# argmaxinc/DiffusionKit

Hardware: NVIDIA H100
Metric: images/sec at 1024x1024 (FLUX.1-schnell 4-step) (higher is better)
Workload: dtype bf16

## Files before the change

### diffusionkit_b200/csrc/common.cuh

```cuda
#pragma once

#include <cuda.h>
#include <cuda_bf16.h>
#include <cuda_fp16.h>
#include <cuda_runtime.h>
#include <stdint.h>
#include <stdio.h>

#include "wgmma.cuh"

namespace dk {

__device__ __forceinline__ uint32_t smem_u32(const void* p) {
  return static_cast<uint32_t>(__cvta_generic_to_shared(p));
}


#ifndef DK_WATCHDOG_CYCLES
#define DK_WATCHDOG_CYCLES (8000000000LL)
#endif

__device__ __forceinline__ void mbar_init(uint64_t* bar, uint32_t count) {
  asm volatile("mbarrier.init.shared::cta.b64 [%0], %1;" ::"r"(smem_u32(bar)), "r"(count) : "memory");
}
// ... 14 lines not shown
      "mbarrier.try_wait.parity.shared::cta.b64 p, [%1], %2;\n\t"
      "selp.u32 %0, 1, 0, p;\n\t}"
      : "=r"(ok)
      : "r"(smem_u32(bar)), "r"(parity)
      : "memory");
  return ok;
}
#ifndef DK_WATCHDOG_SPINS
#define DK_WATCHDOG_SPINS (1u << 26)
#endif
static __device__ __noinline__ void mbar_watchdog_trap(uint64_t* bar, uint32_t parity) {
  printf("[dkb200] mbarrier watchdog: block (%d,%d,%d) thread %d bar@%u parity %u\n", blockIdx.x, blockIdx.y, blockIdx.z,
         threadIdx.x, smem_u32(bar), parity);
  __trap();
}
__device__ __forceinline__ void mbar_wait(uint64_t* bar, uint32_t parity) {
  if (mbar_try_wait(bar, parity)) return;
  uint32_t spins = 0;
  while (!mbar_try_wait(bar, parity)) {
    if (++spins == DK_WATCHDOG_SPINS) mbar_watchdog_trap(bar, parity);
  }
}


__device__ __forceinline__ void mbar_wait_warp(uint64_t* bar, uint32_t parity) {
  if ((threadIdx.x & 31) == 0) mbar_wait(bar, parity);
  __syncwarp();
}

__device__ __forceinline__ void fence_proxy_async_smem() {
  asm volatile("fence.proxy.async.shared::cta;" ::: "memory");
}

__device__ __forceinline__ void named_bar_sync(uint32_t id, uint32_t nthreads) {
  asm volatile("bar.sync %0, %1;" ::"r"(id), "r"(nthreads) : "memory");
}

__device__ __forceinline__ void tma_prefetch_desc(const CUtensorMap* m) {
  asm volatile("prefetch.tensormap [%0];" ::"l"(reinterpret_cast<uint64_t>(m)) : "memory");
}
__device__ __forceinline__ void tma_load_2d(void* dst, const CUtensorMap* map, uint64_t* bar, int c0, int c1) {
  asm volatile(
      "cp.async.bulk.tensor.2d.shared::cluster.global.tile.mbarrier::complete_tx::bytes [%0], [%1, {%3, %4}], [%2];" ::
          "r"(smem_u32(dst)),
      "l"(reinterpret_cast<uint64_t>(map)), "r"(smem_u32(bar)), "r"(c0), "r"(c1)
      : "memory");
}
__device__ __forceinline__ void tma_load_4d(void* dst, const CUtensorMap* map, uint64_t* bar, int c0, int c1, int c2,
                                            int c3) {
  asm volatile(
      "cp.async.bulk.tensor.4d.shared::cluster.global.tile.mbarrier::complete_tx::bytes [%0], [%1, {%3, %4, %5, %6}], "
      "[%2];" ::"r"(smem_u32(dst)),
      "l"(reinterpret_cast<uint64_t>(map)), "r"(smem_u32(bar)), "r"(c0), "r"(c1), "r"(c2), "r"(c3)
      : "memory");
}

__device__ __forceinline__ void wgmma_fence() { asm volatile("wgmma.fence.sync.aligned;" ::: "memory"); }
__device__ __forceinline__ void wgmma_commit() { asm volatile("wgmma.commit_group.sync.aligned;" ::: "memory"); }
template <int N>
__device__ __forceinline__ void wgmma_wait() {
  asm volatile("wgmma.wait_group.sync.aligned %0;" ::"n"(N) : "memory");
}
template <int N>
__device__ __forceinline__ void reg_fence(float (&d)[N]) {
#pragma unroll
  for (int i = 0; i < N; ++i) asm volatile("" : "+f"(d[i])::"memory");
}

// ... 104 lines not shown
```

### diffusionkit_b200/csrc/gemm.cu

```cuda
#include <stdlib.h>

#include "common.cuh"
#include "gemm_epilogue.cuh"
#include "host.h"

namespace dk {

constexpr int BM = 128;
constexpr int BK = 64;
constexpr int GEMM_THREADS = 384;

template <int BN>
struct GemmCfg {
  static constexpr int STAGES = (BN == 256) ? 4 : (BN == 128 ? 6 : 8);
  static constexpr int A_BYTES = BM * BK * 2;
  static constexpr int B_BYTES = BN * BK * 2;
  static constexpr int PIPE_BYTES = STAGES * (A_BYTES + B_BYTES);
  static constexpr int STAGE_LD = BN + 4;
  static_assert(PIPE_BYTES >= BM * STAGE_LD * 4, "the epilogue staging tile reuses the pipeline buffers");
  static constexpr int BAR_BYTES = 256;
  static constexpr int SMEM_BYTES = PIPE_BYTES + BAR_BYTES + 1024;
};

template <typename T, int BN, bool B_MN, int MODE>
__global__ void __launch_bounds__(GEMM_THREADS, 1)
gemm_wgmma_kernel(const __grid_constant__ CUtensorMap tmA, const __grid_constant__ CUtensorMap tmB, const GemmShape s,
                  const GemmEpi e, const ConvGeom g) {
  using Cfg = GemmCfg<BN>;
  constexpr int STAGES = Cfg::STAGES;
  constexpr int A_BYTES = Cfg::A_BYTES;
  constexpr int B_BYTES = Cfg::B_BYTES;

  extern __shared__ uint8_t smem_raw[];
  uint8_t* smem = smem_raw + ((1024u - (smem_u32(smem_raw) & 1023u)) & 1023u);
  uint8_t* sA = smem;
  uint8_t* sB = smem + STAGES * A_BYTES;
  uint64_t* full_bar = reinterpret_cast<uint64_t*>(smem + Cfg::PIPE_BYTES);
  uint64_t* empty_bar = full_bar + STAGES;

  const int warp = threadIdx.x >> 5;
  const int lane = threadIdx.x & 31;
  const int wg = threadIdx.x >> 7;

  if (threadIdx.x == 0) {
    tma_prefetch_desc(&tmA);
    tma_prefetch_desc(&tmB);
    for (int i = 0; i < STAGES; ++i) {
      mbar_init(&full_bar[i], 1);
      mbar_init(&empty_bar[i], 8);
    }
    fence_barrier_init();
  }
  __syncthreads();

  constexpr int GM = 16;
  int m_blk, n_blk;
  {
    const int tile = blockIdx.x;
    const int group_size = GM * s.num_n;
    const int group = tile / group_size;
    const int first_m = group * GM;
    const int gsz = min(s.num_m - first_m, GM);
    const int in_group = tile - group * group_size;
    m_blk = first_m + in_group % gsz;
    n_blk = in_group / gsz;
  }

  if (wg == 0) {
    if (warp != 0) return;
    int img = 0, y0 = 0, x0 = 0;
    if (MODE == 1) {
      const int per_img = g.tiles_x * g.tiles_y;
      img = m_blk / per_img;
      const int t = m_blk - img * per_img;
      y0 = (t / g.tiles_x) * g.TH;
      x0 = (t % g.tiles_x) * g.TW;
    }
    uint32_t stage = 0, phase = 0;
    for (int kb = 0; kb < s.num_k; ++kb) {
      mbar_wait_warp(&empty_bar[stage], phase ^ 1);
      if (elect_one_sync()) {
        mbar_arrive_expect_tx(&full_bar[stage], A_BYTES + B_BYTES);
        uint8_t* a_dst = sA + stage * A_BYTES;
        uint8_t* b_dst = sB + stage * B_BYTES;
        if (MODE == 0) {
          tma_load_2d(a_dst, &tmA, &full_bar[stage], kb * BK, m_blk * BM);
        } else {
          const int tap = kb / g.cblocks;
          const int c0 = (kb - tap * g.cblocks) * BK;
          const int dy = tap / 3, dx = tap - dy * 3;
          tma_load_4d(a_dst, &tmA, &full_bar[stage], c0, x0 * g.stride + dx - g.pad, y0 * g.stride + dy - g.pad, img);
        }
        if (!B_MN) {
          tma_load_2d(b_dst, &tmB, &full_bar[stage], kb * BK, n_blk * BN);
        } else {
#pragma unroll
          for (int j = 0; j < BN / 64; ++j)
            tma_load_2d(b_dst + j * (BK * 128), &tmB, &full_bar[stage], n_blk * BN + j * 64, kb * BK);
        }
      }
      __syncwarp();
      if (++stage == STAGES) {
        stage = 0;
        phase ^= 1;
      }
    }
    return;
  }

  const int cw = wg - 1;
  float acc[BN / 2];
#pragma unroll
  for (int i = 0; i < BN / 2; ++i) acc[i] = 0.f;
  {
    uint32_t stage = 0, phase = 0, prev = 0;
    for (int kb = 0; kb < s.num_k; ++kb) {
      mbar_wait(&full_bar[stage], phase);
      const uint32_t a_base = smem_u32(sA + stage * A_BYTES) + cw * 64 * 128;
      const uint32_t b_base = smem_u32(sB + stage * B_BYTES);
      wgmma_fence();
#pragma unroll
      for (int k = 0; k < BK / 16; ++k) {
        const uint64_t da = make_smem_desc_sw128(a_base + k * 32, 16, 1024);
        const uint64_t db = B_MN ? make_smem_desc_sw128(b_base + k * 16 * 128, BK * 128, 1024)
                                 : make_smem_desc_sw128(b_base + k * 32, 16, 1024);
        Wgmma<BN, Half16<T>::is_bf16, B_MN ? 1 : 0>::ss(acc, da, db, (kb | k) != 0 ? 1u : 0u);
      }
      wgmma_commit();
      wgmma_wait<1>();
      if (kb > 0 && lane == 0) mbar_arrive(&empty_bar[prev]);
      prev = stage;
      if (++stage == STAGES) {
        stage = 0;
        phase ^= 1;
      }
    }
    wgmma_wait<0>();
    reg_fence(acc);
  }

  float* stg = reinterpret_cast<float*>(smem);
  named_bar_sync(1, 256);
  stage_acc_rows<BN>(stg, Cfg::STAGE_LD, cw * 64, acc);
  named_bar_sync(1, 256);

  const int ew = warp - 4;
  const int quarter = ew & 3;
  const int half = ew >> 2;
  constexpr int NCH = BN / 64;
  const int r_in_tile = quarter * 32 + lane;

  bool row_ok;
  long long orow, rrow;
  int batch, pos = 0;
  if (MODE == 0) {
    const int m = m_blk * BM + r_in_tile;
    row_ok = m < s.M;
    batch = m / e.rpb;
    const int in_b = m - batch * e.rpb;
    pos = e.out_row_off + in_b;
    orow = static_cast<long long>(batch) * e.out_batch_rows + e.out_row_off + in_b;
    rrow = static_cast<long long>(batch) * e.res_batch_rows + e.res_row_off + in_b;
  } else {
    const int per_img = g.tiles_x * g.tiles_y;
    const int img = m_blk / per_img;
    const int t = m_blk - img * per_img;
    const int y = (t / g.tiles_x) * g.TH + r_in_tile / g.TW;
    const int x = (t % g.tiles_x) * g.TW + r_in_tile % g.TW;
    row_ok = (y < g.H) && (x < g.W);
    batch = img;
    orow = (static_cast<long long>(img) * g.H + y) * g.W + x;
    rrow = orow;
  }
  const float* srow = stg + r_in_tile * Cfg::STAGE_LD + half * (BN / 2);
  auto load32 = [&](int c, uint32_t (&r)[32]) {
#pragma unroll
    for (int q = 0; q < 8; ++q) {
      const float4 v = *reinterpret_cast<const float4*>(srow + c + 4 * q);
      r[4 * q] = __float_as_uint(v.x);
      r[4 * q + 1] = __float_as_uint(v.y);
      r[4 * q + 2] = __float_as_uint(v.z);
      r[4 * q + 3] = __float_as_uint(v.w);
    }
  };
  gemm_epilogue_drain<T, NCH, MODE>(s, e, load32, n_blk * BN + half * (BN / 2), row_ok, orow, rrow, batch, pos);
}

template <typename T, int BN, bool B_MN, int MODE>
static int launch_gemm_inst(dk_ctx* ctx, const CUtensorMap& tmA, const CUtensorMap& tmB, const GemmShape& s,
                            const GemmEpi& e, const ConvGeom& g, cudaStream_t stream) {
  using Cfg = GemmCfg<BN>;
  auto kern = gemm_wgmma_kernel<T, BN, B_MN, MODE>;
  static bool configured = false;
  if (!configured) {
    DK_CHECK_CUDA(cudaFuncSetAttribute(kern, cudaFuncAttributeMaxDynamicSharedMemorySize, Cfg::SMEM_BYTES));
    configured = true;
  }
  kern<<<s.num_m * s.num_n, GEMM_THREADS, Cfg::SMEM_BYTES, stream>>>(tmA, tmB, s, e, g);
  DK_LAUNCH_CHECK(ctx);
  return 0;
}

template <typename T, bool B_MN, int MODE>
static int launch_gemm_bn(dk_ctx* ctx, int bn, const CUtensorMap& tmA, const CUtensorMap& tmB, const GemmShape& s,
                          const GemmEpi& e, const ConvGeom& g, cudaStream_t stream) {
  if (bn == 256) return launch_gemm_inst<T, 256, B_MN, MODE>(ctx, tmA, tmB, s, e, g, stream);
  if (bn == 128) return launch_gemm_inst<T, 128, B_MN, MODE>(ctx, tmA, tmB, s, e, g, stream);
  return launch_gemm_inst<T, 64, B_MN, MODE>(ctx, tmA, tmB, s, e, g, stream);
}

static int pick_bn(const dk_ctx* ctx, int num_m, int N) {
  if (N <= 64) return 64;
  if (N <= 128) return 128;
  const int tiles256 = num_m * dk_ceil_div(N, 256);
  if (tiles256 >= ctx->sm_count) return 256;
  const int tiles128 = num_m * dk_ceil_div(N, 128);
  if (tiles128 >= ctx->sm_count || N % 256 != 0) return 128;
  return (tiles256 * 2 > ctx->sm_count) ? 256 : 128;
}

static bool aligned16(const void* p) { return (reinterpret_cast<uintptr_t>(p) & 15u) == 0; }
// ... 18 lines not shown
  GemmShape s = {};
  s.M = a->M;
  s.N = a->N;
  s.K = a->K;
  s.num_m = dk_ceil_div(a->M, BM);
  s.num_k = dk_ceil_div(a->K, BK);
  const int bn = a->w_n_major ? 128 : (a->qk_head_dim != 0 ? 256 : pick_bn(ctx, s.num_m, a->N));
  s.num_n = dk_ceil_div(a->N, bn);

  GemmEpi e;
  e.out = a->out;
  e.ldc = a->ldc;
  e.bias = a->bias;
  e.gate = a->gate;
  e.gate_ld = a->gate_ld;
  e.res = a->res;
  e.ldres = a->ldres;
  e.rpb = a->rows_per_batch > 0 ? a->rows_per_batch : a->M;
  e.out_batch_rows = a->rows_per_batch > 0 ? a->out_batch_rows : a->M;
  e.out_row_off = a->out_row_off;
  e.res_batch_rows = a->rows_per_batch > 0 ? a->res_batch_rows : a->M;
  e.res_row_off = a->res_row_off;
  e.act = a->act;
  {
    static const int dbg = [] { const char* v = getenv("DK_GEMM_EPI_DEBUG"); return v ? atoi(v) : 0; }();
    e.debug = dbg;
  }
  e.qk_qw = a->qk_q_weight;
  e.qk_kw = a->qk_k_weight;
  e.qk_rope = a->qk_rope;
  e.qk_d = a->qk_head_dim;
  e.qk_h = a->qk_heads * a->qk_head_dim;
  e.qk_eps = a->qk_eps;
  if (e.qk_d != 0) {
    DK_REQUIRE(e.qk_d == 64 || e.qk_d == 128, "dk_gemm: fused QK norm/RoPE supports head dims 64 and 128 (got %d)", e.qk_d);
    DK_REQUIRE(a->N == 3 * e.qk_h && e.qk_h % 128 == 0, "dk_gemm: fused QK epilogue needs N == 3*heads*d, heads*d %% 128 == 0");
    DK_REQUIRE(!a->w_n_major && a->act == DK_ACT_NONE && a->gate == nullptr && a->res == nullptr,
               "dk_gemm: fused QK epilogue excludes act/gate/residual");
    DK_REQUIRE(a->qk_rope == nullptr || (reinterpret_cast<uintptr_t>(a->qk_rope) & 15u) == 0, "dk_gemm: rope table alignment");
  }
  ConvGeom g = {};

  CUtensorMap tmA, tmB;
  {
    const uint64_t dims[2] = {static_cast<uint64_t>(a->K), static_cast<uint64_t>(a->M)};
    const uint64_t strides[1] = {static_cast<uint64_t>(a->lda) * 2};
    const uint32_t box[2] = {BK, BM};
    if (int rc = dk_make_tmap_16b(ctx, &tmA, a->A, 2, dims, strides, box)) return rc;
  }
  if (!a->w_n_major) {
    const uint64_t dims[2] = {static_cast<uint64_t>(a->K), static_cast<uint64_t>(a->N)};
    const uint64_t strides[1] = {static_cast<uint64_t>(a->ldw) * 2};
    const uint32_t box[2] = {BK, static_cast<uint32_t>(bn)};
    if (int rc = dk_make_tmap_16b(ctx, &tmB, a->W, 2, dims, strides, box)) return rc;
  } else {
    const uint64_t dims[2] = {static_cast<uint64_t>(a->N), static_cast<uint64_t>(a->K)};
    const uint64_t strides[1] = {static_cast<uint64_t>(a->ldw) * 2};
    const uint32_t box[2] = {64, BK};
    if (int rc = dk_make_tmap_16b(ctx, &tmB, a->W, 2, dims, strides, box)) return rc;
  }

  if (a->dtype == DK_BF16) {
    if (a->w_n_major) return launch_gemm_inst<__nv_bfloat16, 128, true, 0>(ctx, tmA, tmB, s, e, g, stream);
    return launch_gemm_bn<__nv_bfloat16, false, 0>(ctx, bn, tmA, tmB, s, e, g, stream);
  } else {
    if (a->w_n_major) return launch_gemm_inst<__half, 128, true, 0>(ctx, tmA, tmB, s, e, g, stream);
    return launch_gemm_bn<__half, false, 0>(ctx, bn, tmA, tmB, s, e, g, stream);
  }
}

static int conv3x3_impl(dk_ctx* ctx, int dtype, const void* x, const void* w, const void* bias, const void* res,
                        void* out, int B, int Hin, int Win, int Cin, int Cout, int stride, cudaStream_t stream) {
  DK_REQUIRE(ctx != nullptr, "dk_conv3x3: null ctx");
  DkDeviceGuard dk_guard_(ctx);
  DK_REQUIRE(dtype == DK_BF16 || dtype == DK_FP16, "dk_conv3x3: bad dtype %d", dtype);
  DK_REQUIRE(B > 0 && Hin > 0 && Win > 0, "dk_conv3x3: empty input");
// ... 35 lines not shown
  GemmEpi e = {};
  e.out = out;
  e.ldc = Cout;
  e.bias = bias;
  e.res = res;
  e.ldres = Cout;
  e.rpb = 1;
  e.act = DK_ACT_NONE;

  CUtensorMap tmA, tmB;
  {
    const uint64_t dims[4] = {static_cast<uint64_t>(Cin), static_cast<uint64_t>(Win), static_cast<uint64_t>(Hin),
                              static_cast<uint64_t>(B)};
    const uint64_t strides[3] = {static_cast<uint64_t>(Cin) * 2, static_cast<uint64_t>(Win) * Cin * 2,
                                 static_cast<uint64_t>(Hin) * Win * Cin * 2};
    const uint32_t box[4] = {BK, static_cast<uint32_t>(g.TW * stride), static_cast<uint32_t>(g.TH * stride), 1};
    const uint32_t estr[4] = {1, static_cast<uint32_t>(stride), static_cast<uint32_t>(stride), 1};
    DK_REQUIRE(box[1] <= 256 && box[2] <= 256, "dk_conv3x3: TMA box too large");
    if (int rc = dk_make_tmap_16b(ctx, &tmA, x, 4, dims, strides, box, estr)) return rc;
  }
  {
    const uint64_t dims[2] = {static_cast<uint64_t>(9 * Cin), static_cast<uint64_t>(Cout)};
    const uint64_t strides[1] = {static_cast<uint64_t>(9 * Cin) * 2};
    const uint32_t box[2] = {BK, static_cast<uint32_t>(bn)};
    if (int rc = dk_make_tmap_16b(ctx, &tmB, w, 2, dims, strides, box)) return rc;
  }
  if (dtype == DK_BF16) return launch_gemm_bn<__nv_bfloat16, false, 1>(ctx, bn, tmA, tmB, s, e, g, stream);
  return launch_gemm_bn<__half, false, 1>(ctx, bn, tmA, tmB, s, e, g, stream);
}

extern "C" int dk_conv3x3(dk_ctx* ctx, int dtype, const void* x, const void* w, const void* bias, const void* res,
                          void* out, int B, int H, int W, int Cin, int Cout, void* stream_) {
  return conv3x3_impl(ctx, dtype, x, w, bias, res, out, B, H, W, Cin, Cout, 1, static_cast<cudaStream_t>(stream_));
}

extern "C" int dk_conv3x3_s2(dk_ctx* ctx, int dtype, const void* x, const void* w, const void* bias, void* out, int B,
                             int H, int W, int Cin, int Cout, void* stream_) {
  return conv3x3_impl(ctx, dtype, x, w, bias, nullptr, out, B, H, W, Cin, Cout, 2, static_cast<cudaStream_t>(stream_));
}
```

### diffusionkit_b200/csrc/gemm_epilogue.cuh

```cuda
#pragma once

#include "common.cuh"
#include "../../include/dkb200.h"

namespace dk {

struct GemmShape {
  int M, N, K;
  int num_m, num_n, num_k;
};

struct GemmEpi {
  void* out;
  long long ldc;
  const void* bias;
  const void* gate;
  long long gate_ld;
  const void* res;
  long long ldres;
  int rpb;
  int out_batch_rows, out_row_off;
  int res_batch_rows, res_row_off;
  int act;
  int debug;
  const void* qk_qw;
  const void* qk_kw;
  const float* qk_rope;
  int qk_h, qk_d;
  float qk_eps;
};

struct ConvGeom {
  int B, H, W, Cin;
  int stride, pad;
  int TH, TW;
  int tiles_x, tiles_y;
  int cblocks;
};


__device__ __forceinline__ void store_row16(void* dst, const uint32_t (&w)[8]) {
  __stcs(reinterpret_cast<uint4*>(dst), make_uint4(w[0], w[1], w[2], w[3]));
  __stcs(reinterpret_cast<uint4*>(dst) + 1, make_uint4(w[4], w[5], w[6], w[7]));
}

template <typename T, int NCH, int MODE, typename Load>
__device__ __forceinline__ void gemm_epilogue_drain(const GemmShape& s, const GemmEpi& e, Load load32, int n_half0,
                                                    bool row_ok, long long orow, long long rrow, int batch, int pos) {
  using H16 = Half16<T>;
  const T* bias = reinterpret_cast<const T*>(e.bias);
  const T* gate = reinterpret_cast<const T*>(e.gate);
  const T* res = reinterpret_cast<const T*>(e.res);
  T* out = reinterpret_cast<T*>(e.out);
  if (MODE == 0 && e.qk_d != 0 && n_half0 < 2 * e.qk_h) {
  const int d = e.qk_d;
  const int cph = d >> 5;
  const T* nw = reinterpret_cast<const T*>(n_half0 < e.qk_h ? e.qk_qw : e.qk_kw);
#pragma unroll 1
  for (int hc = 0; hc < NCH; hc += cph) {
    float ss = 0.f;
    if (nw != nullptr) {
#pragma unroll 1
      for (int c = 0; c < cph; ++c) {
        uint32_t r[32];
        load32((hc + c) * 32, r);
        const int n0 = n_half0 + (hc + c) * 32;
#pragma unroll
        for (int j = 0; j < 4; ++j) {
          float bv[8];
#pragma unroll
          for (int i = 0; i < 8; ++i) bv[i] = 0.f;
          if (bias != nullptr) {
            const uint4 b4 = *reinterpret_cast<const uint4*>(bias + n0 + j * 8);
            const uint32_t bw[4] = {b4.x, b4.y, b4.z, b4.w};
#pragma unroll
            for (int i = 0; i < 4; ++i) {
              const float2 f = H16::unpack(bw[i]);
              bv[2 * i] = f.x;
              bv[2 * i + 1] = f.y;
            }
          }
#pragma unroll
          for (int i = 0; i < 8; ++i) {
            const float v = H16::to_f(H16::from_f(__uint_as_float(r[j * 8 + i]) + bv[i]));
            ss += v * v;
          }
        }
      }
    }
    const float rstd = rsqrtf(ss / d + e.qk_eps);
    const int head_col0 = (n_half0 + hc * 32) % d;
#pragma unroll 1
    for (int c = 0; c < cph; ++c) {
      uint32_t r[32];
      load32((hc + c) * 32, r);
      if (!row_ok || e.debug >= 2) continue;
      const int n0 = n_half0 + (hc + c) * 32;
      const int dcol0 = head_col0 + c * 32;
      uint32_t w16[8];
#pragma unroll
      for (int j = 0; j < 4; ++j) {
        const int n = n0 + j * 8;
        float v[8];
#pragma unroll
        for (int i = 0; i < 8; ++i) v[i] = __uint_as_float(r[j * 8 + i]);
        if (bias != nullptr) {
          const uint4 b4 = *reinterpret_cast<const uint4*>(bias + n);
          const uint32_t bw[4] = {b4.x, b4.y, b4.z, b4.w};
#pragma unroll
          for (int i = 0; i < 4; ++i) {
            const float2 f = H16::unpack(bw[i]);
            v[2 * i] += f.x;
            v[2 * i + 1] += f.y;
          }
        }
        if (nw != nullptr) {
          const uint4 w4 = *reinterpret_cast<const uint4*>(nw + dcol0 + j * 8);
          const uint32_t ww[4] = {w4.x, w4.y, w4.z, w4.w};
#pragma unroll
          for (int i = 0; i < 4; ++i) {
            const float2 f = H16::unpack(ww[i]);
            v[2 * i] = H16::to_f(H16::from_f(H16::to_f(H16::from_f(v[2 * i])) * rstd * f.x));
            v[2 * i + 1] = H16::to_f(H16::from_f(H16::to_f(H16::from_f(v[2 * i + 1])) * rstd * f.y));
          }
        }
        if (e.qk_rope != nullptr) {
          const float4* rp = reinterpret_cast<const float4*>(
              e.qk_rope + (static_cast<long long>(pos) * (d >> 1) + ((dcol0 + j * 8) >> 1)) * 2);
#pragma unroll
          for (int i = 0; i < 2; ++i) {
            const float4 cs = rp[i];
            const float a0 = v[4 * i], a1 = v[4 * i + 1], b0 = v[4 * i + 2], b1 = v[4 * i + 3];
            v[4 * i] = a0 * cs.x - a1 * cs.y;
            v[4 * i + 1] = a0 * cs.y + a1 * cs.x;
            v[4 * i + 2] = b0 * cs.z - b1 * cs.w;
            v[4 * i + 3] = b0 * cs.w + b1 * cs.z;
          }
        }
#pragma unroll
        for (int i = 0; i < 4; ++i) w16[(j & 1) * 4 + i] = H16::pack(v[2 * i], v[2 * i + 1]);
        if ((j & 1) && e.debug == 0) {
          T* dst = out + orow * e.ldc + (n - 8);
          store_row16(dst, w16);
        }
      }
    }
  }
  return;
}

#pragma unroll 1
for (int chunk = 0; chunk < NCH; ++chunk) {
  uint32_t r[32];
  load32(chunk * 32, r);
  const int n0 = n_half0 + chunk * 32;
  if (!row_ok || e.debug >= 2) continue;
#pragma unroll
  for (int j16 = 0; j16 < 2; ++j16) {
    const int nb = n0 + j16 * 16;
    if (nb >= s.N) break;
    uint32_t w[8];
#pragma unroll
    for (int hh = 0; hh < 2; ++hh) {
      const int j = j16 * 2 + hh;
      const int n = n0 + j * 8;
      float v[8];
#pragma unroll
      for (int i = 0; i < 8; ++i) v[i] = __uint_as_float(r[j * 8 + i]);
      if (n < s.N) {
        if (bias != nullptr) {
          const uint4 b4 = *reinterpret_cast<const uint4*>(bias + n);
          const uint32_t bw[4] = {b4.x, b4.y, b4.z, b4.w};
#pragma unroll
          for (int i = 0; i < 4; ++i) {
            const float2 f = H16::unpack(bw[i]);
            v[2 * i] += f.x;
            v[2 * i + 1] += f.y;
          }
        }
        if (e.act == DK_ACT_GELU_ERF) {
#pragma unroll
          for (int i = 0; i < 8; ++i) v[i] = gelu_erf(v[i]);
        } else if (e.act == DK_ACT_SILU) {
#pragma unroll
          for (int i = 0; i < 8; ++i) v[i] = silu_f(v[i]);
        } else if (e.act == DK_ACT_QUICK_GELU) {
#pragma unroll
          for (int i = 0; i < 8; ++i) v[i] = quick_gelu_f(v[i]);
        }
        if (gate != nullptr) {
          const uint4 g4 = *reinterpret_cast<const uint4*>(gate + static_cast<long long>(batch) * e.gate_ld + n);
          const uint32_t gw[4] = {g4.x, g4.y, g4.z, g4.w};
#pragma unroll
          for (int i = 0; i < 4; ++i) {
            const float2 f = H16::unpack(gw[i]);
            v[2 * i] *= f.x;
            v[2 * i + 1] *= f.y;
          }
        }
        if (res != nullptr) {
          const uint4 r4 = *reinterpret_cast<const uint4*>(res + rrow * e.ldres + n);
          const uint32_t rw[4] = {r4.x, r4.y, r4.z, r4.w};
#pragma unroll
          for (int i = 0; i < 4; ++i) {
            const float2 f = H16::unpack(rw[i]);
            v[2 * i] += f.x;
            v[2 * i + 1] += f.y;
          }
        }
      }
#pragma unroll
      for (int i = 0; i < 4; ++i) w[hh * 4 + i] = H16::pack(v[2 * i], v[2 * i + 1]);
    }
    if (e.debug != 0) continue;
    T* dst = out + orow * e.ldc + nb;
    if (nb + 16 <= s.N) {
      store_row16(dst, w);
    } else {
      __stcs(reinterpret_cast<uint4*>(dst), make_uint4(w[0], w[1], w[2], w[3]));
    }
  }
}
}

}
```

Before: 1.673.

## Make GEMM persistent with 2-CTA clusters, B-tile multicast, and register-direct epilogue

The GEMM kernel becomes persistent: a grid sized to the number of resident 2-CTA clusters loops over cluster tiles. The two CTAs in a cluster share each weight (B) tile through TMA multicast, each loading half, and empty barriers are signalled across the cluster. Producer and consumer warpgroups rebalance registers with setmaxnreg. The epilogue is rewritten to work per consumer warpgroup straight from accumulator registers into a dedicated swizzled staging buffer, replacing the old full-tile fp32 staging and the debug path. This is meant to cut B-operand L2 traffic, launch and tail overhead, and the epilogue barrier cost, at the price of more complex synchronisation and shared-memory use.

```diff
diff --git a/diffusionkit_b200/csrc/common.cuh b/diffusionkit_b200/csrc/common.cuh
--- a/diffusionkit_b200/csrc/common.cuh
+++ b/diffusionkit_b200/csrc/common.cuh
@@ -60,18 +60,45 @@
   }
 }
 
+__device__ __forceinline__ void mbar_wait_nocall(uint64_t* bar, uint32_t parity) {
+  uint32_t spins = 0;
+  while (!mbar_try_wait(bar, parity)) {
+    if (++spins == DK_WATCHDOG_SPINS) asm volatile("trap;");
+  }
+}
 
 __device__ __forceinline__ void mbar_wait_warp(uint64_t* bar, uint32_t parity) {
   if ((threadIdx.x & 31) == 0) mbar_wait(bar, parity);
   __syncwarp();
 }
 
+__device__ __forceinline__ void st_shared_u32(uint32_t addr, uint32_t v) {
+  asm volatile("st.shared.u32 [%0], %1;" ::"r"(addr), "r"(v));
+}
+
 __device__ __forceinline__ void fence_proxy_async_smem() {
   asm volatile("fence.proxy.async.shared::cta;" ::: "memory");
 }
 
 __device__ __forceinline__ void named_bar_sync(uint32_t id, uint32_t nthreads) {
   asm volatile("bar.sync %0, %1;" ::"r"(id), "r"(nthreads) : "memory");
+}
+
+__device__ __forceinline__ uint32_t cluster_ctarank() {
+  uint32_t r;
+  asm volatile("mov.u32 %0, %%cluster_ctarank;" : "=r"(r));
+  return r;
+}
+__device__ __forceinline__ void cluster_sync() {
+  asm volatile("barrier.cluster.arrive.release;\n\tbarrier.cluster.wait.acquire;" ::: "memory");
+}
+__device__ __forceinline__ void mbar_arrive_cluster(uint64_t* bar, uint32_t cta) {
+  asm volatile(
+      "{\n\t.reg .b32 ra;\n\t"
+      "mapa.shared::cluster.u32 ra, %0, %1;\n\t"
+      "mbarrier.arrive.shared::cluster.b64 _, [ra];\n\t}" ::"r"(smem_u32(bar)),
+      "r"(cta)
+      : "memory");
 }
 
 __device__ __forceinline__ void tma_prefetch_desc(const CUtensorMap* m) {
@@ -82,6 +109,14 @@
       "cp.async.bulk.tensor.2d.shared::cluster.global.tile.mbarrier::complete_tx::bytes [%0], [%1, {%3, %4}], [%2];" ::
           "r"(smem_u32(dst)),
       "l"(reinterpret_cast<uint64_t>(map)), "r"(smem_u32(bar)), "r"(c0), "r"(c1)
+      : "memory");
+}
+__device__ __forceinline__ void tma_load_2d_multicast(void* dst, const CUtensorMap* map, uint64_t* bar, int c0, int c1,
+                                                      uint16_t cta_mask) {
+  asm volatile(
+      "cp.async.bulk.tensor.2d.shared::cluster.global.tile.mbarrier::complete_tx::bytes.multicast::cluster "
+      "[%0], [%1, {%3, %4}], [%2], %5;" ::"r"(smem_u32(dst)),
+      "l"(reinterpret_cast<uint64_t>(map)), "r"(smem_u32(bar)), "r"(c0), "r"(c1), "h"(cta_mask)
       : "memory");
 }
 __device__ __forceinline__ void tma_load_4d(void* dst, const CUtensorMap* map, uint64_t* bar, int c0, int c1, int c2,
diff --git a/diffusionkit_b200/csrc/gemm.cu b/diffusionkit_b200/csrc/gemm.cu
--- a/diffusionkit_b200/csrc/gemm.cu
+++ b/diffusionkit_b200/csrc/gemm.cu
@@ -1,4 +1,4 @@
-#include <stdlib.h>
+#include <algorithm>
 
 #include "common.cuh"
 #include "gemm_epilogue.cuh"
@@ -9,6 +9,7 @@
 constexpr int BM = 128;
 constexpr int BK = 64;
 constexpr int GEMM_THREADS = 384;
+constexpr int CLUSTER = 2;
 
 template <int BN>
 struct GemmCfg {
@@ -16,11 +17,24 @@
   static constexpr int A_BYTES = BM * BK * 2;
   static constexpr int B_BYTES = BN * BK * 2;
   static constexpr int PIPE_BYTES = STAGES * (A_BYTES + B_BYTES);
-  static constexpr int STAGE_LD = BN + 4;
-  static_assert(PIPE_BYTES >= BM * STAGE_LD * 4, "the epilogue staging tile reuses the pipeline buffers");
+  static constexpr int EPI_BYTES = BM * (BN < 128 ? BN : 128) * 2;
+  static constexpr int RSTD_BYTES = BM * 2 * 4;
   static constexpr int BAR_BYTES = 256;
-  static constexpr int SMEM_BYTES = PIPE_BYTES + BAR_BYTES + 1024;
+  static constexpr int SMEM_BYTES = PIPE_BYTES + EPI_BYTES + RSTD_BYTES + BAR_BYTES + 1024;
+  static_assert(SMEM_BYTES <= 227 * 1024, "shared memory per block");
 };
+
+__device__ __forceinline__ void cluster_tile(int ct, const GemmShape& s, uint32_t rank, int& m_blk, int& n_blk) {
+  constexpr int GC = 8;
+  const int num_cm = (s.num_m + 1) >> 1;
+  const int group_size = GC * s.num_n;
+  const int group = ct / group_size;
+  const int first = group * GC;
+  const int gsz = min(num_cm - first, GC);
+  const int in_group = ct - group * group_size;
+  m_blk = 2 * (first + in_group % gsz) + static_cast<int>(rank);
+  n_blk = in_group / gsz;
+}
 
 template <typename T, int BN, bool B_MN, int MODE>
 __global__ void __launch_bounds__(GEMM_THREADS, 1)
@@ -35,155 +49,126 @@
   uint8_t* smem = smem_raw + ((1024u - (smem_u32(smem_raw) & 1023u)) & 1023u);
   uint8_t* sA = smem;
   uint8_t* sB = smem + STAGES * A_BYTES;
-  uint64_t* full_bar = reinterpret_cast<uint64_t*>(smem + Cfg::PIPE_BYTES);
+  uint8_t* stg = smem + Cfg::PIPE_BYTES;
+  float* rstd = reinterpret_cast<float*>(stg + Cfg::EPI_BYTES);
+  uint64_t* full_bar = reinterpret_cast<uint64_t*>(stg + Cfg::EPI_BYTES + Cfg::RSTD_BYTES);
   uint64_t* empty_bar = full_bar + STAGES;
 
   const int warp = threadIdx.x >> 5;
   const int lane = threadIdx.x & 31;
   const int wg = threadIdx.x >> 7;
+  const uint32_t rank = cluster_ctarank();
 
   if (threadIdx.x == 0) {
     tma_prefetch_desc(&tmA);
     tma_prefetch_desc(&tmB);
     for (int i = 0; i < STAGES; ++i) {
       mbar_init(&full_bar[i], 1);
-      mbar_init(&empty_bar[i], 8);
+      mbar_init(&empty_bar[i], 8 * CLUSTER);
     }
     fence_barrier_init();
   }
-  __syncthreads();
-
-  constexpr int GM = 16;
-  int m_blk, n_blk;
-  {
-    const int tile = blockIdx.x;
-    const int group_size = GM * s.num_n;
-    const int group = tile / group_size;
-    const int first_m = group * GM;
-    const int gsz = min(s.num_m - first_m, GM);
-    const int in_group = tile - group * group_size;
-    m_blk = first_m + in_group % gsz;
-    n_blk = in_group / gsz;
-  }
+  cluster_sync();
+
+  const int num_ctiles = ((s.num_m + 1) >> 1) * s.num_n;
+  const int first_ct = blockIdx.x / CLUSTER;
+  const int ct_stride = gridDim.x / CLUSTER;
 
   if (wg == 0) {
-    if (warp != 0) return;
-    int img = 0, y0 = 0, x0 = 0;
-    if (MODE == 1) {
-      const int per_img = g.tiles_x * g.tiles_y;
-      img = m_blk / per_img;
-      const int t = m_blk - img * per_img;
-      y0 = (t / g.tiles_x) * g.TH;
-      x0 = (t % g.tiles_x) * g.TW;
-    }
-    uint32_t stage = 0, phase = 0;
-    for (int kb = 0; kb < s.num_k; ++kb) {
-      mbar_wait_warp(&empty_bar[stage], phase ^ 1);
-      if (elect_one_sync()) {
-        mbar_arrive_expect_tx(&full_bar[stage], A_BYTES + B_BYTES);
-        uint8_t* a_dst = sA + stage * A_BYTES;
-        uint8_t* b_dst = sB + stage * B_BYTES;
-        if (MODE == 0) {
-          tma_load_2d(a_dst, &tmA, &full_bar[stage], kb * BK, m_blk * BM);
-        } else {
-          const int tap = kb / g.cblocks;
-          const int c0 = (kb - tap * g.cblocks) * BK;
-          const int dy = tap / 3, dx = tap - dy * 3;
-          tma_load_4d(a_dst, &tmA, &full_bar[stage], c0, x0 * g.stride + dx - g.pad, y0 * g.stride + dy - g.pad, img);
-        }
-        if (!B_MN) {
-          tma_load_2d(b_dst, &tmB, &full_bar[stage], kb * BK, n_blk * BN);
-        } else {
+    setmaxnreg_dec<40>();
+    if (warp == 0) {
+      uint32_t stage = 0, phase = 0;
+      for (int ct = first_ct; ct < num_ctiles; ct += ct_stride) {
+        int m_blk, n_blk;
+        cluster_tile(ct, s, rank, m_blk, n_blk);
+        int img = 0, y0 = 0, x0 = 0;
+        if (MODE == 1) {
+          const int per_img = g.tiles_x * g.tiles_y;
+          img = m_blk / per_img;
+          const int t = m_blk - img * per_img;
+          y0 = (t / g.tiles_x) * g.TH;
+          x0 = (t % g.tiles_x) * g.TW;
+        }
+        for (int kb = 0; kb < s.num_k; ++kb) {
+          if (lane == 0) mbar_wait_nocall(&empty_bar[stage], phase ^ 1);
+          __syncwarp();
+          if (elect_one_sync()) {
+            mbar_arrive_expect_tx(&full_bar[stage], A_BYTES + B_BYTES);
+            uint8_t* a_dst = sA + stage * A_BYTES;
+            uint8_t* b_dst = sB + stage * B_BYTES;
+            if (MODE == 0) {
+              tma_load_2d(a_dst, &tmA, &full_bar[stage], kb * BK, m_blk * BM);
+            } else {
+              const int tap = kb / g.cblocks;
+              const int c0 = (kb - tap * g.cblocks) * BK;
+              const int dy = tap / 3, dx = tap - dy * 3;
+              tma_load_4d(a_dst, &tmA, &full_bar[stage], c0, x0 * g.stride + dx - g.pad, y0 * g.stride + dy - g.pad,
+                          img);
+            }
+            if (!B_MN) {
+              tma_load_2d_multicast(b_dst + rank * (B_BYTES / 2), &tmB, &full_bar[stage], kb * BK,
+                                    n_blk * BN + static_cast<int>(rank) * (BN / 2), 0x3);
+            } else {
 #pragma unroll
-          for (int j = 0; j < BN / 64; ++j)
-            tma_load_2d(b_dst + j * (BK * 128), &tmB, &full_bar[stage], n_blk * BN + j * 64, kb * BK);
-        }
-      }
-      __syncwarp();
-      if (++stage == STAGES) {
-        stage = 0;
-        phase ^= 1;
+              for (int j = 0; j < BN / 64; ++j)
+                if (j % CLUSTER == static_cast<int>(rank))
+                  tma_load_2d_multicast(b_dst + j * (BK * 128), &tmB, &full_bar[stage], n_blk * BN + j * 64, kb * BK,
+                                        0x3);
+            }
+          }
+          __syncwarp();
+          if (++stage == STAGES) {
+            stage = 0;
+            phase ^= 1;
+          }
+        }
       }
     }
-    return;
-  }
-
-  const int cw = wg - 1;
-  float acc[BN / 2];
+  } else {
+    setmaxnreg_inc<232>();
+    const int cw = wg - 1;
+    float acc[BN / 2];
 #pragma unroll
-  for (int i = 0; i < BN / 2; ++i) acc[i] = 0.f;
-  {
-    uint32_t stage = 0, phase = 0, prev = 0;
-    for (int kb = 0; kb < s.num_k; ++kb) {
-      mbar_wait(&full_bar[stage], phase);
-      const uint32_t a_base = smem_u32(sA + stage * A_BYTES) + cw * 64 * 128;
-      const uint32_t b_base = smem_u32(sB + stage * B_BYTES);
-      wgmma_fence();
+    for (int i = 0; i < BN / 2; ++i) acc[i] = 0.f;
+    uint32_t stage = 0, phase = 0;
+    for (int ct = first_ct; ct < num_ctiles; ct += ct_stride) {
+      int m_blk, n_blk;
+      cluster_tile(ct, s, rank, m_blk, n_blk);
+      uint32_t prev = 0;
+      for (int kb = 0; kb < s.num_k; ++kb) {
+        mbar_wait_nocall(&full_bar[stage], phase);
+        const uint32_t a_base = smem_u32(sA + stage * A_BYTES) + cw * 64 * 128;
+        const uint32_t b_base = smem_u32(sB + stage * B_BYTES);
+        wgmma_fence();
 #pragma unroll
-      for (int k = 0; k < BK / 16; ++k) {
-        const uint64_t da = make_smem_desc_sw128(a_base + k * 32, 16, 1024);
-        const uint64_t db = B_MN ? make_smem_desc_sw128(b_base + k * 16 * 128, BK * 128, 1024)
-                                 : make_smem_desc_sw128(b_base + k * 32, 16, 1024);
-        Wgmma<BN, Half16<T>::is_bf16, B_MN ? 1 : 0>::ss(acc, da, db, (kb | k) != 0 ? 1u : 0u);
+        for (int k = 0; k < BK / 16; ++k) {
+          const uint64_t da = make_smem_desc_sw128(a_base + k * 32, 16, 1024);
+          const uint64_t db = B_MN ? make_smem_desc_sw128(b_base + k * 16 * 128, BK * 128, 1024)
+                                   : make_smem_desc_sw128(b_base + k * 32, 16, 1024);
+          Wgmma<BN, Half16<T>::is_bf16, B_MN ? 1 : 0>::ss(acc, da, db, (kb | k) != 0 ? 1u : 0u);
+        }
+        wgmma_commit();
+        wgmma_wait<1>();
+        if (kb > 0 && lane == 0) {
+          mbar_arrive_cluster(&empty_bar[prev], 0);
+          mbar_arrive_cluster(&empty_bar[prev], 1);
+        }
+        prev = stage;
+        if (++stage == STAGES) {
+          stage = 0;
+          phase ^= 1;
+        }
       }
-      wgmma_commit();
-      wgmma_wait<1>();
-      if (kb > 0 && lane == 0) mbar_arrive(&empty_bar[prev]);
-      prev = stage;
-      if (++stage == STAGES) {
-        stage = 0;
-        phase ^= 1;
+      wgmma_wait<0>();
+      reg_fence(acc);
+      if (lane == 0) {
+        mbar_arrive_cluster(&empty_bar[prev], 0);
+        mbar_arrive_cluster(&empty_bar[prev], 1);
       }
+      gemm_epilogue_tile<T, BN, MODE>(acc, s, e, g, m_blk, n_blk, cw, stg + cw * (Cfg::EPI_BYTES / 2), rstd + cw * 128);
     }
-    wgmma_wait<0>();
-    reg_fence(acc);
-  }
-
-  float* stg = reinterpret_cast<float*>(smem);
-  named_bar_sync(1, 256);
-  stage_acc_rows<BN>(stg, Cfg::STAGE_LD, cw * 64, acc);
-  named_bar_sync(1, 256);
-
-  const int ew = warp - 4;
-  const int quarter = ew & 3;
-  const int half = ew >> 2;
-  constexpr int NCH = BN / 64;
-  const int r_in_tile = quarter * 32 + lane;
-
-  bool row_ok;
-  long long orow, rrow;
-  int batch, pos = 0;
-  if (MODE == 0) {
-    const int m = m_blk * BM + r_in_tile;
-    row_ok = m < s.M;
-    batch = m / e.rpb;
-    const int in_b = m - batch * e.rpb;
-    pos = e.out_row_off + in_b;
-    orow = static_cast<long long>(batch) * e.out_batch_rows + e.out_row_off + in_b;
-    rrow = static_cast<long long>(batch) * e.res_batch_rows + e.res_row_off + in_b;
-  } else {
-    const int per_img = g.tiles_x * g.tiles_y;
-    const int img = m_blk / per_img;
-    const int t = m_blk - img * per_img;
-    const int y = (t / g.tiles_x) * g.TH + r_in_tile / g.TW;
-    const int x = (t % g.tiles_x) * g.TW + r_in_tile % g.TW;
-    row_ok = (y < g.H) && (x < g.W);
-    batch = img;
-    orow = (static_cast<long long>(img) * g.H + y) * g.W + x;
-    rrow = orow;
-  }
-  const float* srow = stg + r_in_tile * Cfg::STAGE_LD + half * (BN / 2);
-  auto load32 = [&](int c, uint32_t (&r)[32]) {
-#pragma unroll
-    for (int q = 0; q < 8; ++q) {
-      const float4 v = *reinterpret_cast<const float4*>(srow + c + 4 * q);
-      r[4 * q] = __float_as_uint(v.x);
-      r[4 * q + 1] = __float_as_uint(v.y);
-      r[4 * q + 2] = __float_as_uint(v.z);
-      r[4 * q + 3] = __float_as_uint(v.w);
-    }
-  };
-  gemm_epilogue_drain<T, NCH, MODE>(s, e, load32, n_blk * BN + half * (BN / 2), row_ok, orow, rrow, batch, pos);
+  }
+  cluster_sync();
 }
 
 template <typename T, int BN, bool B_MN, int MODE>
@@ -191,12 +176,29 @@
                             const GemmEpi& e, const ConvGeom& g, cudaStream_t stream) {
   using Cfg = GemmCfg<BN>;
   auto kern = gemm_wgmma_kernel<T, BN, B_MN, MODE>;
-  static bool configured = false;
-  if (!configured) {
+  cudaLaunchAttribute cluster;
+  cluster.id = cudaLaunchAttributeClusterDimension;
+  cluster.val.clusterDim.x = CLUSTER;
+  cluster.val.clusterDim.y = 1;
+  cluster.val.clusterDim.z = 1;
+  cudaLaunchConfig_t cfg = {};
+  cfg.gridDim = dim3(CLUSTER);
+  cfg.blockDim = dim3(GEMM_THREADS);
+  cfg.dynamicSmemBytes = Cfg::SMEM_BYTES;
+  cfg.stream = stream;
+  cfg.attrs = &cluster;
+  cfg.numAttrs = 1;
+  static int max_clusters = 0;
+  if (max_clusters == 0) {
     DK_CHECK_CUDA(cudaFuncSetAttribute(kern, cudaFuncAttributeMaxDynamicSharedMemorySize, Cfg::SMEM_BYTES));
-    configured = true;
-  }
-  kern<<<s.num_m * s.num_n, GEMM_THREADS, Cfg::SMEM_BYTES, stream>>>(tmA, tmB, s, e, g);
+    int n = 0;
+    DK_CHECK_CUDA(cudaOccupancyMaxActiveClusters(&n, kern, &cfg));
+    DK_REQUIRE(n > 0, "dk_gemm: no 2-CTA cluster of the GEMM kernel fits on the device");
+    max_clusters = n;
+  }
+  const int cluster_tiles = dk_ceil_div(s.num_m, CLUSTER) * s.num_n;
+  cfg.gridDim = dim3(CLUSTER * std::min(cluster_tiles, max_clusters));
+  DK_CHECK_CUDA(cudaLaunchKernelEx(&cfg, kern, tmA, tmB, s, e, g));
   DK_LAUNCH_CHECK(ctx);
   return 0;
 }
@@ -261,10 +263,6 @@
   e.res_batch_rows = a->rows_per_batch > 0 ? a->res_batch_rows : a->M;
   e.res_row_off = a->res_row_off;
   e.act = a->act;
-  {
-    static const int dbg = [] { const char* v = getenv("DK_GEMM_EPI_DEBUG"); return v ? atoi(v) : 0; }();
-    e.debug = dbg;
-  }
   e.qk_qw = a->qk_q_weight;
   e.qk_kw = a->qk_k_weight;
   e.qk_rope = a->qk_rope;
@@ -290,7 +288,7 @@
   if (!a->w_n_major) {
     const uint64_t dims[2] = {static_cast<uint64_t>(a->K), static_cast<uint64_t>(a->N)};
     const uint64_t strides[1] = {static_cast<uint64_t>(a->ldw) * 2};
-    const uint32_t box[2] = {BK, static_cast<uint32_t>(bn)};
+    const uint32_t box[2] = {BK, static_cast<uint32_t>(bn / CLUSTER)};
     if (int rc = dk_make_tmap_16b(ctx, &tmB, a->W, 2, dims, strides, box)) return rc;
   } else {
     const uint64_t dims[2] = {static_cast<uint64_t>(a->N), static_cast<uint64_t>(a->K)};
@@ -372,7 +370,7 @@
   {
     const uint64_t dims[2] = {static_cast<uint64_t>(9 * Cin), static_cast<uint64_t>(Cout)};
     const uint64_t strides[1] = {static_cast<uint64_t>(9 * Cin) * 2};
-    const uint32_t box[2] = {BK, static_cast<uint32_t>(bn)};
+    const uint32_t box[2] = {BK, static_cast<uint32_t>(bn / CLUSTER)};
     if (int rc = dk_make_tmap_16b(ctx, &tmB, w, 2, dims, strides, box)) return rc;
   }
   if (dtype == DK_BF16) return launch_gemm_bn<__nv_bfloat16, false, 1>(ctx, bn, tmA, tmB, s, e, g, stream);
diff --git a/diffusionkit_b200/csrc/gemm_epilogue.cuh b/diffusionkit_b200/csrc/gemm_epilogue.cuh
--- a/diffusionkit_b200/csrc/gemm_epilogue.cuh
+++ b/diffusionkit_b200/csrc/gemm_epilogue.cuh
@@ -22,7 +22,6 @@
   int out_batch_rows, out_row_off;
   int res_batch_rows, res_row_off;
   int act;
-  int debug;
   const void* qk_qw;
   const void* qk_kw;
   const float* qk_rope;
@@ -38,189 +37,288 @@
   int cblocks;
 };
 
-
-__device__ __forceinline__ void store_row16(void* dst, const uint32_t (&w)[8]) {
-  __stcs(reinterpret_cast<uint4*>(dst), make_uint4(w[0], w[1], w[2], w[3]));
-  __stcs(reinterpret_cast<uint4*>(dst) + 1, make_uint4(w[4], w[5], w[6], w[7]));
+struct EpiRow {
+  bool ok;
+  int batch, pos;
+  long long orow, rrow;
+};
+template <int MODE>
+__device__ __forceinline__ EpiRow epi_row(const GemmShape& s, const GemmEpi& e, const ConvGeom& g, int m_blk, int r) {
+  EpiRow o;
+  if (MODE == 0) {
+    const int m = m_blk * 128 + r;
+    o.ok = m < s.M;
+    o.batch = m / e.rpb;
+    const int in_b = m - o.batch * e.rpb;
+    o.pos = e.out_row_off + in_b;
+    o.orow = static_cast<long long>(o.batch) * e.out_batch_rows + e.out_row_off + in_b;
+    o.rrow = static_cast<long long>(o.batch) * e.res_batch_rows + e.res_row_off + in_b;
+  } else {
+    const int per_img = g.tiles_x * g.tiles_y;
+    const int img = m_blk / per_img;
+    const int t = m_blk - img * per_img;
+    const int y = (t / g.tiles_x) * g.TH + r / g.TW;
+    const int x = (t % g.tiles_x) * g.TW + r % g.TW;
+    o.ok = img < g.B && y < g.H && x < g.W;
+    o.batch = img;
+    o.pos = 0;
+    o.orow = (static_cast<long long>(img) * g.H + y) * g.W + x;
+    o.rrow = o.orow;
+  }
+  return o;
 }
 
-template <typename T, int NCH, int MODE, typename Load>
-__device__ __forceinline__ void gemm_epilogue_drain(const GemmShape& s, const GemmEpi& e, Load load32, int n_half0,
-                                                    bool row_ok, long long orow, long long rrow, int batch, int pos) {
+template <typename T>
+__device__ __forceinline__ uint32_t ld_u32(const T* p) {
+  return *reinterpret_cast<const uint32_t*>(p);
+}
+
+template <typename T, int BN, int MODE>
+__device__ __forceinline__ void gemm_epilogue_tile(const float (&acc)[BN / 2], const GemmShape& s, const GemmEpi& e,
+                                                   const ConvGeom& g, int m_blk, int n_blk, int cw, uint8_t* stg,
+                                                   float* rstd) {
   using H16 = Half16<T>;
+  constexpr int EC = BN < 128 ? BN : 128;
+  constexpr int JP = EC / 8;
+  constexpr int ROWB = EC * 2;
+  constexpr int G = 4;
+  constexpr int GQ = 2;
+  const uint32_t bar = 1 + cw;
+  const int t = threadIdx.x & 127;
+  const int lane = t & 31;
+  const int q = lane & 3;
+  const int rl0 = (t >> 5) * 16 + (lane >> 2);
+  const int row0 = cw * 64;
   const T* bias = reinterpret_cast<const T*>(e.bias);
   const T* gate = reinterpret_cast<const T*>(e.gate);
   const T* res = reinterpret_cast<const T*>(e.res);
   T* out = reinterpret_cast<T*>(e.out);
-  if (MODE == 0 && e.qk_d != 0 && n_half0 < 2 * e.qk_h) {
-  const int d = e.qk_d;
-  const int cph = d >> 5;
-  const T* nw = reinterpret_cast<const T*>(n_half0 < e.qk_h ? e.qk_qw : e.qk_kw);
+  auto slot = [&](int rl, int jj) { return rl * ROWB + ((jj ^ (rl & 7)) << 4) + q * 4; };
+  const uint32_t stg_s = smem_u32(stg);
+  auto put = [&](int rl, int jj, float lo, float hi) { st_shared_u32(stg_s + slot(rl, jj), H16::pack(lo, hi)); };
+
+#pragma unroll
+  for (int p = 0; p < BN / EC; ++p) {
+    const int n_pass = n_blk * BN + p * EC;
+    if (MODE == 0 && e.qk_d != 0 && n_pass < 2 * e.qk_h) {
+      const int d = e.qk_d;
+      const EpiRow fr[2] = {epi_row<MODE>(s, e, g, m_blk, row0 + rl0), epi_row<MODE>(s, e, g, m_blk, row0 + rl0 + 8)};
+      const T* nw = reinterpret_cast<const T*>(n_pass < e.qk_h ? e.qk_qw : e.qk_kw);
+      const float* rope[2];
+#pragma unroll
+      for (int i = 0; i < 2; ++i)
+        rope[i] = e.qk_rope + (fr[i].ok ? static_cast<long long>(fr[i].pos) * d : 0);
+      if (nw != nullptr) {
+#pragma unroll
+        for (int j0 = 0; j0 < JP; j0 += G) {
+          uint32_t bw[G];
+          if (bias != nullptr) {
+#pragma unroll
+            for (int u = 0; u < G; ++u) bw[u] = ld_u32(bias + n_pass + 8 * (j0 + u) + 2 * q);
+          }
+#pragma unroll
+          for (int u = 0; u < G; ++u) {
+            const int a = p * (EC / 2) + 4 * (j0 + u);
+#pragma unroll
+            for (int i = 0; i < 2; ++i) {
+              float v0 = acc[a + 2 * i], v1 = acc[a + 2 * i + 1];
+              if (bias != nullptr) {
+                const float2 b = H16::unpack(bw[u]);
+                v0 += b.x;
+                v1 += b.y;
+              }
+              put(rl0 + 8 * i, j0 + u, v0, v1);
+            }
+          }
+        }
+        named_bar_sync(bar, 128);
+        if (t < 64 * (EC / d)) {
+          const int rl = t & 63, hd = t >> 6;
+          const int cph = d >> 3;
+          float ss = 0.f;
 #pragma unroll 1
-  for (int hc = 0; hc < NCH; hc += cph) {
-    float ss = 0.f;
-    if (nw != nullptr) {
-#pragma unroll 1
-      for (int c = 0; c < cph; ++c) {
-        uint32_t r[32];
-        load32((hc + c) * 32, r);
-        const int n0 = n_half0 + (hc + c) * 32;
-#pragma unroll
-        for (int j = 0; j < 4; ++j) {
-          float bv[8];
-#pragma unroll
-          for (int i = 0; i < 8; ++i) bv[i] = 0.f;
-          if (bias != nullptr) {
-            const uint4 b4 = *reinterpret_cast<const uint4*>(bias + n0 + j * 8);
-            const uint32_t bw[4] = {b4.x, b4.y, b4.z, b4.w};
-#pragma unroll
-            for (int i = 0; i < 4; ++i) {
-              const float2 f = H16::unpack(bw[i]);
-              bv[2 * i] = f.x;
-              bv[2 * i + 1] = f.y;
-            }
-          }
-#pragma unroll
-          for (int i = 0; i < 8; ++i) {
-            const float v = H16::to_f(H16::from_f(__uint_as_float(r[j * 8 + i]) + bv[i]));
-            ss += v * v;
-          }
-        }
+          for (int c = 0; c < cph; ++c) {
+            const uint4 v4 = *reinterpret_cast<const uint4*>(stg + rl * ROWB + (((hd * cph + c) ^ (rl & 7)) << 4));
+            const uint32_t w[4] = {v4.x, v4.y, v4.z, v4.w};
+#pragma unroll
+            for (int k = 0; k < 4; ++k) {
+              const float2 f = H16::unpack(w[k]);
+              ss += f.x * f.x;
+              ss += f.y * f.y;
+            }
+          }
+          rstd[hd * 64 + rl] = rsqrtf(ss / d + e.qk_eps);
+        }
+        named_bar_sync(bar, 128);
+      }
+#pragma unroll
+      for (int j0 = 0; j0 < JP; j0 += GQ) {
+        uint32_t bw[GQ], ww[GQ];
+        float2 cs[2][GQ];
+        if (nw != nullptr) {
+#pragma unroll
+          for (int u = 0; u < GQ; ++u) ww[u] = ld_u32(nw + ((8 * (j0 + u) + 2 * q) & (d - 1)));
+        } else if (bias != nullptr) {
+#pragma unroll
+          for (int u = 0; u < GQ; ++u) bw[u] = ld_u32(bias + n_pass + 8 * (j0 + u) + 2 * q);
+        }
+        if (e.qk_rope != nullptr) {
+#pragma unroll
+          for (int u = 0; u < GQ; ++u)
+#pragma unroll
+            for (int i = 0; i < 2; ++i)
+              cs[i][u] = *reinterpret_cast<const float2*>(rope[i] + ((8 * (j0 + u) + 2 * q) & (d - 1)));
+        }
+        float v[GQ][2][2];
+        if (nw != nullptr) {
+#pragma unroll
+          for (int u = 0; u < GQ; ++u) {
+            const int hd = 8 * (j0 + u) >= d ? 1 : 0;
+            const float2 w = H16::unpack(ww[u]);
+#pragma unroll
+            for (int i = 0; i < 2; ++i) {
+              const float2 h = H16::unpack(*reinterpret_cast<const uint32_t*>(stg + slot(rl0 + 8 * i, j0 + u)));
+              const float r = rstd[hd * 64 + rl0 + 8 * i];
+              v[u][i][0] = H16::to_f(H16::from_f(h.x * r * w.x));
+              v[u][i][1] = H16::to_f(H16::from_f(h.y * r * w.y));
+            }
+          }
+        } else {
+#pragma unroll
+          for (int u = 0; u < GQ; ++u)
+#pragma unroll
+            for (int i = 0; i < 2; ++i) {
+              const int a = p * (EC / 2) + 4 * (j0 + u) + 2 * i;
+              v[u][i][0] = acc[a];
+              v[u][i][1] = acc[a + 1];
+              if (bias != nullptr) {
+                const float2 b = H16::unpack(bw[u]);
+                v[u][i][0] += b.x;
+                v[u][i][1] += b.y;
+              }
+            }
+        }
+        if (e.qk_rope != nullptr) {
+#pragma unroll
+          for (int u = 0; u < GQ; ++u)
+#pragma unroll
+            for (int i = 0; i < 2; ++i) {
+              const float a0 = v[u][i][0], a1 = v[u][i][1];
+              v[u][i][0] = a0 * cs[i][u].x - a1 * cs[i][u].y;
+              v[u][i][1] = a0 * cs[i][u].y + a1 * cs[i][u].x;
+            }
+        }
+#pragma unroll
+        for (int u = 0; u < GQ; ++u)
+#pragma unroll
+          for (int i = 0; i < 2; ++i) put(rl0 + 8 * i, j0 + u, v[u][i][0], v[u][i][1]);
+      }
+    } else {
+      const EpiRow fr[2] = {epi_row<MODE>(s, e, g, m_blk, row0 + rl0), epi_row<MODE>(s, e, g, m_blk, row0 + rl0 + 8)};
+      const T* grow[2];
+      const T* rrow[2];
+#pragma unroll
+      for (int i = 0; i < 2; ++i) {
+        grow[i] = gate + (fr[i].ok ? static_cast<long long>(fr[i].batch) * e.gate_ld : 0);
+        rrow[i] = res + (fr[i].ok ? fr[i].rrow * e.ldres : 0);
+      }
+#pragma unroll
+      for (int j0 = 0; j0 < JP; j0 += G) {
+        uint32_t bw[G], gw[2][G], rw[2][G];
+        int n[G];
+#pragma unroll
+        for (int u = 0; u < G; ++u) n[u] = min(n_pass + 8 * (j0 + u), s.N - 8) + 2 * q;
+        if (bias != nullptr) {
+#pragma unroll
+          for (int u = 0; u < G; ++u) bw[u] = ld_u32(bias + n[u]);
+        }
+        if (gate != nullptr) {
+#pragma unroll
+          for (int u = 0; u < G; ++u)
+#pragma unroll
+            for (int i = 0; i < 2; ++i) gw[i][u] = ld_u32(grow[i] + n[u]);
+        }
+        if (res != nullptr) {
+#pragma unroll
+          for (int u = 0; u < G; ++u)
+#pragma unroll
+            for (int i = 0; i < 2; ++i) rw[i][u] = ld_u32(rrow[i] + n[u]);
+        }
+        float v[G][2][2];
+#pragma unroll
+        for (int u = 0; u < G; ++u)
+#pragma unroll
+          for (int i = 0; i < 2; ++i) {
+            const int a = p * (EC / 2) + 4 * (j0 + u) + 2 * i;
+            v[u][i][0] = acc[a];
+            v[u][i][1] = acc[a + 1];
+          }
+        if (bias != nullptr) {
+#pragma unroll
+          for (int u = 0; u < G; ++u)
+#pragma unroll
+            for (int i = 0; i < 2; ++i) {
+              const float2 b = H16::unpack(bw[u]);
+              v[u][i][0] += b.x;
+              v[u][i][1] += b.y;
+            }
+        }
+        if (e.act == DK_ACT_GELU_ERF) {
+#pragma unroll
+          for (int u = 0; u < G; ++u)
+#pragma unroll
+            for (int k = 0; k < 4; ++k) v[u][k >> 1][k & 1] = gelu_erf(v[u][k >> 1][k & 1]);
+        } else if (e.act == DK_ACT_SILU) {
+#pragma unroll
+          for (int u = 0; u < G; ++u)
+#pragma unroll
+            for (int k = 0; k < 4; ++k) v[u][k >> 1][k & 1] = silu_f(v[u][k >> 1][k & 1]);
+        } else if (e.act == DK_ACT_QUICK_GELU) {
+#pragma unroll
+          for (int u = 0; u < G; ++u)
+#pragma unroll
+            for (int k = 0; k < 4; ++k) v[u][k >> 1][k & 1] = quick_gelu_f(v[u][k >> 1][k & 1]);
+        }
+        if (gate != nullptr) {
+#pragma unroll
+          for (int u = 0; u < G; ++u)
+#pragma unroll
+            for (int i = 0; i < 2; ++i) {
+              const float2 gv = H16::unpack(gw[i][u]);
+              v[u][i][0] *= gv.x;
+              v[u][i][1] *= gv.y;
+            }
+        }
+        if (res != nullptr) {
+#pragma unroll
+          for (int u = 0; u < G; ++u)
+#pragma unroll
+            for (int i = 0; i < 2; ++i) {
+              const float2 rv = H16::unpack(rw[i][u]);
+              v[u][i][0] += rv.x;
+              v[u][i][1] += rv.y;
+            }
+        }
+#pragma unroll
+        for (int u = 0; u < G; ++u)
+#pragma unroll
+          for (int i = 0; i < 2; ++i) put(rl0 + 8 * i, j0 + u, v[u][i][0], v[u][i][1]);
       }
     }
-    const float rstd = rsqrtf(ss / d + e.qk_eps);
-    const int head_col0 = (n_half0 + hc * 32) % d;
-#pragma unroll 1
-    for (int c = 0; c < cph; ++c) {
-      uint32_t r[32];
-      load32((hc + c) * 32, r);
-      if (!row_ok || e.debug >= 2) continue;
-      const int n0 = n_half0 + (hc + c) * 32;
-      const int dcol0 = head_col0 + c * 32;
-      uint32_t w16[8];
-#pragma unroll
-      for (int j = 0; j < 4; ++j) {
-        const int n = n0 + j * 8;
-        float v[8];
-#pragma unroll
-        for (int i = 0; i < 8; ++i) v[i] = __uint_as_float(r[j * 8 + i]);
-        if (bias != nullptr) {
-          const uint4 b4 = *reinterpret_cast<const uint4*>(bias + n);
-          const uint32_t bw[4] = {b4.x, b4.y, b4.z, b4.w};
-#pragma unroll
-          for (int i = 0; i < 4; ++i) {
-            const float2 f = H16::unpack(bw[i]);
-            v[2 * i] += f.x;
-            v[2 * i + 1] += f.y;
-          }
-        }
-        if (nw != nullptr) {
-          const uint4 w4 = *reinterpret_cast<const uint4*>(nw + dcol0 + j * 8);
-          const uint32_t ww[4] = {w4.x, w4.y, w4.z, w4.w};
-#pragma unroll
-          for (int i = 0; i < 4; ++i) {
-            const float2 f = H16::unpack(ww[i]);
-            v[2 * i] = H16::to_f(H16::from_f(H16::to_f(H16::from_f(v[2 * i])) * rstd * f.x));
-            v[2 * i + 1] = H16::to_f(H16::from_f(H16::to_f(H16::from_f(v[2 * i + 1])) * rstd * f.y));
-          }
-        }
-        if (e.qk_rope != nullptr) {
-          const float4* rp = reinterpret_cast<const float4*>(
-              e.qk_rope + (static_cast<long long>(pos) * (d >> 1) + ((dcol0 + j * 8) >> 1)) * 2);
-#pragma unroll
-          for (int i = 0; i < 2; ++i) {
-            const float4 cs = rp[i];
-            const float a0 = v[4 * i], a1 = v[4 * i + 1], b0 = v[4 * i + 2], b1 = v[4 * i + 3];
-            v[4 * i] = a0 * cs.x - a1 * cs.y;
-            v[4 * i + 1] = a0 * cs.y + a1 * cs.x;
-            v[4 * i + 2] = b0 * cs.z - b1 * cs.w;
-            v[4 * i + 3] = b0 * cs.w + b1 * cs.z;
-          }
-        }
-#pragma unroll
-        for (int i = 0; i < 4; ++i) w16[(j & 1) * 4 + i] = H16::pack(v[2 * i], v[2 * i + 1]);
-        if ((j & 1) && e.debug == 0) {
-          T* dst = out + orow * e.ldc + (n - 8);
-          store_row16(dst, w16);
-        }
-      }
+    named_bar_sync(bar, 128);
+
+    const int c = t % JP;
+    const int n = n_pass + 8 * c;
+#pragma unroll 2
+    for (int r0 = 0; r0 < 64; r0 += 128 / JP) {
+      const int rl = r0 + t / JP;
+      const EpiRow row = epi_row<MODE>(s, e, g, m_blk, row0 + rl);
+      if (row.ok && n < s.N)
+        __stcs(reinterpret_cast<uint4*>(out + row.orow * e.ldc + n),
+               *reinterpret_cast<const uint4*>(stg + rl * ROWB + ((c ^ (rl & 7)) << 4)));
     }
-  }
-  return;
-}
-
-#pragma unroll 1
-for (int chunk = 0; chunk < NCH; ++chunk) {
-  uint32_t r[32];
-  load32(chunk * 32, r);
-  const int n0 = n_half0 + chunk * 32;
-  if (!row_ok || e.debug >= 2) continue;
-#pragma unroll
-  for (int j16 = 0; j16 < 2; ++j16) {
-    const int nb = n0 + j16 * 16;
-    if (nb >= s.N) break;
-    uint32_t w[8];
-#pragma unroll
-    for (int hh = 0; hh < 2; ++hh) {
-      const int j = j16 * 2 + hh;
-      const int n = n0 + j * 8;
-      float v[8];
-#pragma unroll
-      for (int i = 0; i < 8; ++i) v[i] = __uint_as_float(r[j * 8 + i]);
-      if (n < s.N) {
-        if (bias != nullptr) {
-          const uint4 b4 = *reinterpret_cast<const uint4*>(bias + n);
-          const uint32_t bw[4] = {b4.x, b4.y, b4.z, b4.w};
-#pragma unroll
-          for (int i = 0; i < 4; ++i) {
-            const float2 f = H16::unpack(bw[i]);
-            v[2 * i] += f.x;
-            v[2 * i + 1] += f.y;
-          }
-        }
-        if (e.act == DK_ACT_GELU_ERF) {
-#pragma unroll
-          for (int i = 0; i < 8; ++i) v[i] = gelu_erf(v[i]);
-        } else if (e.act == DK_ACT_SILU) {
-#pragma unroll
-          for (int i = 0; i < 8; ++i) v[i] = silu_f(v[i]);
-        } else if (e.act == DK_ACT_QUICK_GELU) {
-#pragma unroll
-          for (int i = 0; i < 8; ++i) v[i] = quick_gelu_f(v[i]);
-        }
-        if (gate != nullptr) {
-          const uint4 g4 = *reinterpret_cast<const uint4*>(gate + static_cast<long long>(batch) * e.gate_ld + n);
-          const uint32_t gw[4] = {g4.x, g4.y, g4.z, g4.w};
-#pragma unroll
-          for (int i = 0; i < 4; ++i) {
-            const float2 f = H16::unpack(gw[i]);
-            v[2 * i] *= f.x;
-            v[2 * i + 1] *= f.y;
-          }
-        }
-        if (res != nullptr) {
-          const uint4 r4 = *reinterpret_cast<const uint4*>(res + rrow * e.ldres + n);
-          const uint32_t rw[4] = {r4.x, r4.y, r4.z, r4.w};
-#pragma unroll
-          for (int i = 0; i < 4; ++i) {
-            const float2 f = H16::unpack(rw[i]);
-            v[2 * i] += f.x;
-            v[2 * i + 1] += f.y;
-          }
-        }
-      }
-#pragma unroll
-      for (int i = 0; i < 4; ++i) w[hh * 4 + i] = H16::pack(v[2 * i], v[2 * i + 1]);
-    }
-    if (e.debug != 0) continue;
-    T* dst = out + orow * e.ldc + nb;
-    if (nb + 16 <= s.N) {
-      store_row16(dst, w);
-    } else {
-      __stcs(reinterpret_cast<uint4*>(dst), make_uint4(w[0], w[1], w[2], w[3]));
-    }
+    named_bar_sync(bar, 128);
   }
 }
+
 }
-
-}
```

Result: faster. 1.816, median of 6 (+8.6%).
